# matpalm/cartpoleplusplus

Hardware: AMD Instinct MI355X
Metric: DDPG training steps/sec, 64x64x18 pixel obs, batch=256 (higher is better)
Workload: dtype f32-acc/f16x2,bf16x6

## Files before the change

cartpoleplusplus_amd/csrc/conv_dw16_rs.h:

```cpp
#pragma once
#include <type_traits>
#include "conv_dw16.h"

template <int CIN_>
struct Dw16RsGeom {
  static constexpr int KS = 5, P = 2, PB = 2, CIN = CIN_, NO = KYO_NO, WC = 32, NPC = 2;
  static constexpr int CP0 = (CIN + 1 + 3) & ~3;
  static constexpr int CP = ((CP0 / 2) % 8 == 0) ? CP0 + 4 : CP0;
  static constexpr bool ODD = (CIN & 1) != 0;
  static constexpr int MT = (KS * CP + 15) / 16, NT = (KS * NO + 15) / 16;
  static constexpr int WPX = WC + 2 * P;
  static constexpr int ROWB = 2 * (((CP * WPX + 16 * MT - KS * CP) + 7) & ~7);
  static constexpr int NXS = 2;
  static constexpr int DOST = 80, DPC = NO * DOST;
  static constexpr int DSLOT = NPC * DPC;
  static constexpr int NDS = KS + 1;
  static constexpr int WVB = NXS * ROWB + NDS * DSLOT;
  static constexpr int SUMB = MT * NT * 64 * 16;
  static constexpr int BASEB = 4 * WVB > 2 * SUMB ? 4 * WVB : 2 * SUMB;
  static constexpr int TXB = NT * KS * 16 * 4;
  static constexpr int LDS_BYTES = (BASEB + 4 * TXB + 2 * CIN * 4 + 15) & ~15;
  static constexpr int NW = KS * KS * CIN * NO;
  static_assert(ROWB % 16 == 0 && WVB % 16 == 0 && BASEB % 16 == 0, "16-byte aligned slots");
  static_assert(MT * NT * 4 <= 112, "the accumulators of a unit: at most 112 registers (18 channels); 30 channels would need 160");
};

template <int CIN_>
__device__ __forceinline__ void conv_dw16_rs_body(const ConvArgsN& batch, const int nbands, const int band, const int bx, const int by) {
  typedef Dw16RsGeom<CIN_> G;
  constexpr int KS = G::KS, P = G::P, PB = G::PB, CIN = G::CIN, NO = G::NO, WC = G::WC, CP = G::CP, MT = G::MT, NT = G::NT, NPC = G::NPC;
  constexpr int ROWB = G::ROWB, DOST = G::DOST, DPC = G::DPC, DSLOT = G::DSLOT, NDS = G::NDS;
  constexpr unsigned BIG = 0x08000000u;
  extern __shared__ __attribute__((aligned(16))) unsigned char dw16rs_lds[];
  const int tid = threadIdx.x, lane = tid & 63, li = lane & 15, lj = lane >> 4;
  const int swave = __builtin_amdgcn_readfirstlane(tid >> 6);
  const int net = swave & 1, col = swave >> 1;
  const ConvArgs& a = batch.a[by + net];
  unsigned char* wvb = dw16rs_lds + swave * G::WVB;
  unsigned char* xring = wvb;
  unsigned char* dzring = wvb + G::NXS * ROWB;
  float* wsc = reinterpret_cast<float*>(dw16rs_lds + G::BASEB + 4 * G::TXB);
  const int H = a.H, Hp = H >> 1, W = a.W, Wp = W >> 1, nout = a.nout;
  const int ub = bx / nbands, bd = bx - ub * nbands;
  const int x0 = col * WC;
  const int q_lo = bd * band;
  const int rows = min(band, H - q_lo);
  const int y0 = q_lo - PB;
  if (tid < CIN) { wsc[tid] = a.scale[tid]; wsc[CIN + tid] = a.shift[tid]; }

  for (int i = lane; i < G::WVB / 16; i += 64) reinterpret_cast<k16_u32x4*>(wvb)[i] = (k16_u32x4){0u, 0u, 0u, 0u};
  for (int i = lane; i < G::NXS * G::WPX; i += 64) {
    const int s = i / G::WPX, wx = i - s * G::WPX, x = x0 - P + wx;
    if (x >= 0 && x < W) *reinterpret_cast<unsigned short*>(xring + s * ROWB + 2 * (CP * wx + CIN)) = (unsigned short)0x3C00u;
  }

  constexpr bool ODDC = G::ODD;
  constexpr int NXV = ODDC ? (G::WPX * CIN / 2 + 63) / 64 : (G::WPX * (CIN / 2) + 63) / 64;
  const __amdgpu_buffer_rsrc_t in_rsrc = __builtin_amdgcn_make_buffer_rsrc(
      const_cast<__half*>((const __half*)a.in + (long)(a.img_slot ? a.img_slot[ub] : ub) * a.in_bstride), 0, H * W * CIN * 2, 0x00020000);
  unsigned xvo[NXV]; uint32_t xdst[NXV]; uint32_t xdst_hi[ODDC ? NXV : 1];
#pragma unroll
  for (int i = 0; i < NXV; ++i) {
    const int idx = lane + 64 * i;
    if (!ODDC) {
      const int wx = idx / (CIN / 2), cp = idx - (CIN / 2) * wx;
      const int x = x0 - P + wx;
      const bool on = idx < G::WPX * (CIN / 2);
      xvo[i] = (on && x >= 0 && x < W) ? (unsigned)((x * CIN + 2 * cp) * 2) : BIG;
      xdst[i] = keep_in_vgpr(lds_addr(xring + (on ? 2 * (CP * wx + 2 * cp) : ROWB - 8)));
    } else {
      const int h0 = 2 * idx, h1 = 2 * idx + 1;
      const int wx0 = h0 / CIN, wx1 = h1 / CIN;
      const int x = x0 - P + wx0;
      const bool on = idx < G::WPX * CIN / 2;
      xvo[i] = (on && x >= 0 && x < W) ? (unsigned)(((x0 - P) * CIN + h0) * 2) : BIG;
      xdst[i] = keep_in_vgpr(lds_addr(xring + (on ? 2 * (CP * wx0 + (h0 - CIN * wx0)) : ROWB - 8)));
      xdst_hi[i] = keep_in_vgpr(lds_addr(xring + (on ? 2 * (CP * wx1 + (h1 - CIN * wx1)) : ROWB - 6)));
    }
  }
  unsigned xraw[2][NXV];
  auto x_load = [&](const int buf, const int q) __attribute__((always_inline)) {
    const unsigned ro = q < H ? (unsigned)(q * (W * CIN * 2)) : BIG;
#pragma unroll
    for (int i = 0; i < NXV; ++i) xraw[buf][i] = __builtin_amdgcn_raw_buffer_load_b32(in_rsrc, (int)(xvo[i] + ro), 0, 0);
  };
  auto x_store = [&](const int buf, const int slot) __attribute__((always_inline)) {
#pragma unroll
    for (int i = 0; i < NXV; ++i) {
      if (!ODDC) lds_store(xdst[i], slot * ROWB, xraw[buf][i]);
      else { lds_store_u16(xdst[i], slot * ROWB, xraw[buf][i] & 0xFFFFu); lds_store_u16(xdst_hi[i], slot * ROWB, xraw[buf][i] >> 16); }
    }
  };

  const int zg = lane / NO, zo = lane - zg * NO;
  const bool zon = lane < 4 * NO;
  const __amdgpu_buffer_rsrc_t dp_rsrc = __builtin_amdgcn_make_buffer_rsrc(const_cast<float*>(a.dy.dpool + (long)ub * a.dy.dpool_bstride), 0,
                                                                           Hp * Wp * NO * 4, 0x00020000);
  const __amdgpu_buffer_rsrc_t am_rsrc = __builtin_amdgcn_make_buffer_rsrc(const_cast<uint8_t*>(a.dy.amax + (long)ub * Hp * Wp * NO), 0,
                                                                           Hp * Wp * NO, 0x00020000);
  const unsigned zoff = zon ? (unsigned)((x0 / 2 + 8 * (zg & 1) + (zg >> 1)) * NO + zo) : BIG;
  const uint32_t zdst = keep_in_vgpr(lds_addr(dzring + (zon ? zo * DOST + zg * 16 : DOST - 16)));

  float sc, inv;
  {
    const int pylo = max(0, (q_lo - P) >> 1), pyhi = min(Hp - 1, (q_lo + rows - 1 + P) >> 1);
    float vmax = 0.f;
    if (a.dy.imax) {
      const f32x4 im = *reinterpret_cast<const f32x4*>(a.dy.imax + (long)ub * DX_IMAX_SLOTS), im2 = *reinterpret_cast<const f32x4*>(a.dy.imax + (long)ub * DX_IMAX_SLOTS + 4);
      vmax = fmaxf(fmaxf(fmaxf(im[0], im[1]), fmaxf(im[2], im[3])), fmaxf(fmaxf(im2[0], im2[1]), fmaxf(im2[2], im2[3])));
    }
    constexpr int PSR = 9;
    for (int py = a.dy.imax ? pyhi + 1 : pylo; py <= pyhi; py += PSR) {
      float t[PSR][4];
#pragma unroll
      for (int u = 0; u < PSR; ++u) {
        const unsigned ro = py + u <= pyhi ? (unsigned)((py + u) * (Wp * NO)) : BIG;
#pragma unroll
        for (int j = 0; j < 4; ++j) t[u][j] = __uint_as_float(__builtin_amdgcn_raw_buffer_load_b32(dp_rsrc, (int)((zoff + ro + (unsigned)(2 * j * NO)) * 4u), 0, 0));
      }
#pragma unroll
      for (int u = 0; u < PSR; ++u)
#pragma unroll
        for (int j = 0; j < 4; ++j) vmax = fmaxf(vmax, fabsf(t[u][j]));
    }
    for (int o = 32; o > 0; o >>= 1) vmax = fmaxf(vmax, __shfl_xor(vmax, o));
    int S = 0;
    if (vmax > 0.f && vmax < 3.0e38f) S = 14 - ilogbf(vmax);
    S = S > 100 ? 100 : (S < -100 ? -100 : S);
    sc = ldexpf(1.f, S); inv = ldexpf(1.f, -S);
  }

  float zrg[2][4]; unsigned zrc[2][4];
#pragma unroll
  for (int b = 0; b < 2; ++b)
#pragma unroll
    for (int j = 0; j < 4; ++j) { zrg[b][j] = 0.f; zrc[b][j] = 0u; }
  unsigned zp01[NPC] = {0u, 0u}, zp23[NPC] = {0u, 0u};
  unsigned zm01[4] = {0u, 0u, 0u, 0u}, zm23[4] = {0u, 0u, 0u, 0u};
  auto z_load = [&](const int buf, const int py) __attribute__((always_inline)) {
    const unsigned ro = (py >= 0 && py < Hp) ? (unsigned)(py * (Wp * NO)) : BIG;
#pragma unroll
    for (int j = 0; j < 4; ++j) {
      const unsigned e = zoff + ro + (unsigned)(2 * j * NO);
      zrg[buf][j] = __uint_as_float(__builtin_amdgcn_raw_buffer_load_b32(dp_rsrc, (int)(e * 4u), 0, 0));
      zrc[buf][j] = (unsigned)__builtin_amdgcn_raw_buffer_load_b8(am_rsrc, (int)e, 0, 0);
    }
  };
  auto z_convert_half = [&](const int buf, const int hf) __attribute__((always_inline)) {
    unsigned short pc[2][NPC];
#pragma unroll
    for (int j = 0; j < 2; ++j) {
      const float g = (zrc[buf][2 * hf + j] & POOL_ACTIVE) ? zrg[buf][2 * hf + j] : 0.f;
      const float v = g * sc;
      const _Float16 h = (_Float16)v;
      const _Float16 m = (_Float16)(v - (float)h);
      pc[j][0] = __builtin_bit_cast(unsigned short, h); pc[j][1] = __builtin_bit_cast(unsigned short, m);
    }
#pragma unroll
    for (int p = 0; p < NPC; ++p) {
      const unsigned v = (unsigned)pc[0][p] | ((unsigned)pc[1][p] << 16);
      if (hf == 0) zp01[p] = v; else zp23[p] = v;
    }
#pragma unroll
    for (int pos = 0; pos < 4; ++pos) {
      const unsigned v = ((zrc[buf][2 * hf] & 3u) == (unsigned)pos ? 0xFFFFu : 0u) | ((zrc[buf][2 * hf + 1] & 3u) == (unsigned)pos ? 0xFFFF0000u : 0u);
      if (hf == 0) zm01[pos] = v; else zm23[pos] = v;
    }
  };
  auto z_convert = [&](const int buf) __attribute__((always_inline)) { z_convert_half(buf, 0); z_convert_half(buf, 1); };
  auto z_store = [&](const int slot, const int ry) __attribute__((always_inline)) {
#pragma unroll
    for (int p = 0; p < NPC; ++p)
      lds_store(zdst, slot * DSLOT + p * DPC, (k16_u32x4){zp01[p] & zm01[2 * ry], zp23[p] & zm23[2 * ry], zp01[p] & zm01[2 * ry + 1], zp23[p] & zm23[2 * ry + 1]});
  };

  const int tj = (lane >> 2) & 3, tq = lane & 3;
  const uint32_t aadr = keep_in_vgpr(lds_addr(xring + 2 * (CP * (16 * (lj & 1) + 4 * tj + 2 * (lj >> 1)) + 4 * tq)));
  uint32_t bbase[NT]; int bky[NT];
#pragma unroll
  for (int nt = 0; nt < NT; ++nt) {
    const int n = 16 * nt + li;
    const bool nvalid = n < KS * NO;
    bky[nt] = nvalid ? n / NO : 0;
    bbase[nt] = lds_addr(dzring + (nvalid ? n % NO : 0) * DOST + lj * 16);
  }
  f32x4 acc[MT][NT];
#pragma unroll
  for (int mt = 0; mt < MT; ++mt)
#pragma unroll
    for (int nt = 0; nt < NT; ++nt) acc[mt][nt] = (f32x4){0.f, 0.f, 0.f, 0.f};

  {
    const int py0 = y0 >> 1;
    z_load(0, py0); z_load(1, py0 + 1);
    x_load(0, q_lo); x_load(1, q_lo + 1);
#pragma unroll
    for (int d = 0; d <= PB + P; ++d) {
      if ((d & 1) == 0) { z_convert((d / 2) % 2); z_load((d / 2) % 2, py0 + d / 2 + 2); }
      z_store(d % NDS, d & 1);
    }
    x_store(0, 0);
    x_load(0, q_lo + 2);
    __builtin_amdgcn_sched_barrier(0);

    k16_u32x4 bq[NT][NPC];
    auto a_load = [&](k16_u32x4& dst, const int xs, const int mt) __attribute__((always_inline)) {
      const int off = xs * ROWB + mt * 32;
      const dw16_v4s r0 = __builtin_amdgcn_ds_read_tr16_b64_v4i16(
          reinterpret_cast<__attribute__((address_space(3))) dw16_v4s*>((uintptr_t)(aadr + (uint32_t)off)));
      const dw16_v4s r1 = __builtin_amdgcn_ds_read_tr16_b64_v4i16(
          reinterpret_cast<__attribute__((address_space(3))) dw16_v4s*>((uintptr_t)(aadr + (uint32_t)(off + 2 * CP))));
      const dw16_u32x2 u0 = __builtin_bit_cast(dw16_u32x2, r0), u1 = __builtin_bit_cast(dw16_u32x2, r1);
      dst = (k16_u32x4){u0.x, u0.y, u1.x, u1.y};
    };
    auto step = [&](auto sqtag, const int t) __attribute__((always_inline)) {
      constexpr int SQ = decltype(sqtag)::value;
      constexpr int XS = SQ & 1;
      constexpr int ZPOS = SQ + PB + P + 1;
      constexpr bool ZODD = (ZPOS & 1) != 0;
      constexpr int ZBUF = (ZPOS / 2) % 2;
#pragma unroll
      for (int nt = 0; nt < NT; ++nt) {
        int sl = (SQ + PB + P) % NDS - bky[nt]; sl = sl < 0 ? sl + NDS : sl;
        const uint32_t ad = bbase[nt] + (uint32_t)(sl * DSLOT);
#pragma unroll
        for (int p = 0; p < NPC; ++p) bq[nt][p] = lds_load<k16_u32x4>(ad, p * DPC);
      }
      k16_u32x4 av;
      a_load(av, XS, 0);
#pragma unroll
      for (int mt = 0; mt < MT; ++mt) {
        k16_u32x4 an = av;
        if (mt + 1 < MT) a_load(an, XS, mt + 1);
#pragma unroll
        for (int pc = NPC - 1; pc >= 0; --pc)
#pragma unroll
          for (int nt = 0; nt < NT; ++nt)
            acc[mt][nt] = __builtin_amdgcn_mfma_f32_16x16x32_f16(__builtin_bit_cast(f16x8, av), __builtin_bit_cast(f16x8, bq[nt][pc]), acc[mt][nt], 0, 0, 0);
        constexpr int TL = MT - 1;
        if (mt == (0 < TL ? 0 : TL)) { if (!ZODD) z_convert_half(ZBUF, 0); }
        if (mt == (1 < TL ? 1 : TL)) { if (!ZODD) z_convert_half(ZBUF, 1); }
        if (mt == (2 < TL ? 2 : TL)) z_store(ZPOS % NDS, ZODD ? 1 : 0);
        if (mt == (3 < TL ? 3 : TL)) { if (ZODD) z_load(ZBUF, py0 + (t + PB + P + 1) / 2 + 2); }
        if (mt == (4 < TL ? 4 : TL)) x_store((SQ + 1) & 1, XS ^ 1);
        if (mt == (5 < TL ? 5 : TL)) x_load((SQ + 1) & 1, q_lo + t + 3);
        av = an;
      }
      __builtin_amdgcn_sched_barrier(0);
    };
    for (int t0 = 0; t0 < rows; t0 += 12) {
      if (t0 + 0 < rows) step(std::integral_constant<int, 0>{}, t0 + 0);
      if (t0 + 1 < rows) step(std::integral_constant<int, 1>{}, t0 + 1);
      if (t0 + 2 < rows) step(std::integral_constant<int, 2>{}, t0 + 2);
      if (t0 + 3 < rows) step(std::integral_constant<int, 3>{}, t0 + 3);
      if (t0 + 4 < rows) step(std::integral_constant<int, 4>{}, t0 + 4);
      if (t0 + 5 < rows) step(std::integral_constant<int, 5>{}, t0 + 5);
      if (t0 + 6 < rows) step(std::integral_constant<int, 6>{}, t0 + 6);
      if (t0 + 7 < rows) step(std::integral_constant<int, 7>{}, t0 + 7);
      if (t0 + 8 < rows) step(std::integral_constant<int, 8>{}, t0 + 8);
      if (t0 + 9 < rows) step(std::integral_constant<int, 9>{}, t0 + 9);
      if (t0 + 10 < rows) step(std::integral_constant<int, 10>{}, t0 + 10);
      if (t0 + 11 < rows) step(std::integral_constant<int, 11>{}, t0 + 11);
    }
  }

  __syncthreads();
  float* sum = reinterpret_cast<float*>(dw16rs_lds + net * G::SUMB);
  if (col == 0) {
#pragma unroll
    for (int mt = 0; mt < MT; ++mt)
#pragma unroll
      for (int nt = 0; nt < NT; ++nt)
        *reinterpret_cast<f32x4*>(sum + ((mt * NT + nt) * 64 + lane) * 4) = (f32x4){acc[mt][nt][0] * inv, acc[mt][nt][1] * inv, acc[mt][nt][2] * inv, acc[mt][nt][3] * inv};
  }
  __syncthreads();
  if (col == 0) return;
#pragma unroll
  for (int mt = 0; mt < MT; ++mt)
#pragma unroll
    for (int nt = 0; nt < NT; ++nt) {
      const f32x4 o = *reinterpret_cast<const f32x4*>(sum + ((mt * NT + nt) * 64 + lane) * 4);
#pragma unroll
      for (int r = 0; r < 4; ++r) acc[mt][nt][r] = o[r] + acc[mt][nt][r] * inv;
    }
  float* tx = reinterpret_cast<float*>(dw16rs_lds + G::BASEB + swave * G::TXB);
#pragma unroll
  for (int nt = 0; nt < NT; ++nt)
#pragma unroll
    for (int kx = 0; kx < KS; ++kx) {
      const int m = CP * kx + CIN;
      if (lj == ((m & 15) >> 2)) tx[(nt * KS + kx) * 16 + li] = acc[m >> 4][nt][m & 3];
    }
  __builtin_amdgcn_fence(__ATOMIC_RELEASE, "wavefront");
  __builtin_amdgcn_wave_barrier();
  __builtin_amdgcn_fence(__ATOMIC_ACQUIRE, "wavefront");
  float* part = a.partial + (long)bx * a.pstride;
#pragma unroll
  for (int nt = 0; nt < NT; ++nt) {
    const int n = 16 * nt + li;
    const bool nvalid = n < KS * NO;
    const int nky = nvalid ? n / NO : 0, no = nvalid ? n % NO : 0;
    if (nvalid && no < nout) {
#pragma unroll
      for (int mt = 0; mt < MT; ++mt)
#pragma unroll
        for (int r = 0; r < 4; ++r) {
          const int m = 16 * mt + 4 * lj + r;
          const int kx = m / CP, c = m - kx * CP;
          if (kx < KS && c < CIN) {
            const float t = tx[(nt * KS + kx) * 16 + li];
            part[(nky * (KS * CIN) + kx * CIN + c) * nout + no] = wsc[c] * acc[mt][nt][r] + wsc[CIN + c] * t;
          } else if (kx == P && c == CIN && nky == P) part[G::NW / NO * nout + no] = acc[mt][nt][r];
        }
    }
  }
}

int conv_dw16_rs_dispatch(cpp_ctx* ctx, int cin, int ks, int in_mode, bool dense, const ConvArgsN& a, int* grid, bool* handled);
```

Baseline: 3185.

## Prefetch next-row B/A fragments across steps and simplify dz packing

```diff
diff --git a/cartpoleplusplus_amd/csrc/conv_dw16_rs.h b/cartpoleplusplus_amd/csrc/conv_dw16_rs.h
--- a/cartpoleplusplus_amd/csrc/conv_dw16_rs.h
+++ b/cartpoleplusplus_amd/csrc/conv_dw16_rs.h
@@ -135,8 +135,11 @@
   for (int b = 0; b < 2; ++b)
 #pragma unroll
     for (int j = 0; j < 4; ++j) { zrg[b][j] = 0.f; zrc[b][j] = 0u; }
-  unsigned zp01[NPC] = {0u, 0u}, zp23[NPC] = {0u, 0u};
-  unsigned zm01[4] = {0u, 0u, 0u, 0u}, zm23[4] = {0u, 0u, 0u, 0u};
+  unsigned long long zw[4][NPC];
+#pragma unroll
+  for (int j = 0; j < 4; ++j)
+#pragma unroll
+    for (int p = 0; p < NPC; ++p) zw[j][p] = 0ull;
   auto z_load = [&](const int buf, const int py) __attribute__((always_inline)) {
     const unsigned ro = (py >= 0 && py < Hp) ? (unsigned)(py * (Wp * NO)) : BIG;
 #pragma unroll
@@ -147,43 +150,41 @@
     }
   };
   auto z_convert_half = [&](const int buf, const int hf) __attribute__((always_inline)) {
-    unsigned short pc[2][NPC];
-#pragma unroll
-    for (int j = 0; j < 2; ++j) {
-      const float g = (zrc[buf][2 * hf + j] & POOL_ACTIVE) ? zrg[buf][2 * hf + j] : 0.f;
+#pragma unroll
+    for (int j = 2 * hf; j < 2 * hf + 2; ++j) {
+      const float g = (zrc[buf][j] & POOL_ACTIVE) ? zrg[buf][j] : 0.f;
       const float v = g * sc;
       const _Float16 h = (_Float16)v;
       const _Float16 m = (_Float16)(v - (float)h);
-      pc[j][0] = __builtin_bit_cast(unsigned short, h); pc[j][1] = __builtin_bit_cast(unsigned short, m);
-    }
-#pragma unroll
-    for (int p = 0; p < NPC; ++p) {
-      const unsigned v = (unsigned)pc[0][p] | ((unsigned)pc[1][p] << 16);
-      if (hf == 0) zp01[p] = v; else zp23[p] = v;
-    }
-#pragma unroll
-    for (int pos = 0; pos < 4; ++pos) {
-      const unsigned v = ((zrc[buf][2 * hf] & 3u) == (unsigned)pos ? 0xFFFFu : 0u) | ((zrc[buf][2 * hf + 1] & 3u) == (unsigned)pos ? 0xFFFF0000u : 0u);
-      if (hf == 0) zm01[pos] = v; else zm23[pos] = v;
+      const unsigned sh = (zrc[buf][j] << 4) & 63u;
+      zw[j][0] = (unsigned long long)__builtin_bit_cast(unsigned short, h) << sh;
+      zw[j][1] = (unsigned long long)__builtin_bit_cast(unsigned short, m) << sh;
     }
   };
   auto z_convert = [&](const int buf) __attribute__((always_inline)) { z_convert_half(buf, 0); z_convert_half(buf, 1); };
   auto z_store = [&](const int slot, const int ry) __attribute__((always_inline)) {
 #pragma unroll
-    for (int p = 0; p < NPC; ++p)
-      lds_store(zdst, slot * DSLOT + p * DPC, (k16_u32x4){zp01[p] & zm01[2 * ry], zp23[p] & zm23[2 * ry], zp01[p] & zm01[2 * ry + 1], zp23[p] & zm23[2 * ry + 1]});
+    for (int p = 0; p < NPC; ++p) {
+      unsigned d[4];
+#pragma unroll
+      for (int k = 0; k < 4; ++k) {
+        const int j = 2 * (k & 1), rx = k >> 1;
+        d[k] = __builtin_amdgcn_perm((unsigned)(zw[j + 1][p] >> (32 * ry)), (unsigned)(zw[j][p] >> (32 * ry)), rx ? 0x07060302u : 0x05040100u);
+      }
+      lds_store(zdst, slot * DSLOT + p * DPC, (k16_u32x4){d[0], d[1], d[2], d[3]});
+    }
   };
 
   const int tj = (lane >> 2) & 3, tq = lane & 3;
   const uint32_t aadr = keep_in_vgpr(lds_addr(xring + 2 * (CP * (16 * (lj & 1) + 4 * tj + 2 * (lj >> 1)) + 4 * tq)));
-  uint32_t bbase[NT]; int bky[NT];
+  uint32_t bring[NT];
 #pragma unroll
   for (int nt = 0; nt < NT; ++nt) {
     const int n = 16 * nt + li;
     const bool nvalid = n < KS * NO;
-    bky[nt] = nvalid ? n / NO : 0;
-    bbase[nt] = lds_addr(dzring + (nvalid ? n % NO : 0) * DOST + lj * 16);
-  }
+    bring[nt] = keep_in_vgpr(lds_addr(dzring + (NDS - (nvalid ? n / NO : 0)) * DSLOT + (nvalid ? n % NO : 0) * DOST + lj * 16));
+  }
+  const uint32_t bend = lds_addr(dzring + NDS * DSLOT);
   f32x4 acc[MT][NT];
 #pragma unroll
   for (int mt = 0; mt < MT; ++mt)
@@ -201,9 +202,14 @@
     }
     x_store(0, 0);
     x_load(0, q_lo + 2);
-    __builtin_amdgcn_sched_barrier(0);
-
-    k16_u32x4 bq[NT][NPC];
+
+    k16_u32x4 bq[NT][NPC], av;
+    auto b_load = [&](const int sq, const int nt) __attribute__((always_inline)) {
+      const uint32_t c = bring[nt] + (uint32_t)(((sq + PB + P) % NDS) * DSLOT);
+      const uint32_t ad = c >= bend ? c - (uint32_t)(NDS * DSLOT) : c;
+#pragma unroll
+      for (int p = 0; p < NPC; ++p) bq[nt][p] = lds_load<k16_u32x4>(ad, p * DPC);
+    };
     auto a_load = [&](k16_u32x4& dst, const int xs, const int mt) __attribute__((always_inline)) {
       const int off = xs * ROWB + mt * 32;
       const dw16_v4s r0 = __builtin_amdgcn_ds_read_tr16_b64_v4i16(
@@ -213,37 +219,57 @@
       const dw16_u32x2 u0 = __builtin_bit_cast(dw16_u32x2, r0), u1 = __builtin_bit_cast(dw16_u32x2, r1);
       dst = (k16_u32x4){u0.x, u0.y, u1.x, u1.y};
     };
+#pragma unroll
+    for (int nt = 0; nt < NT; ++nt) b_load(0, nt);
+    a_load(av, 0, 0);
+    __builtin_amdgcn_sched_barrier(0);
+
+    auto mfma = [&](const int mt, const int nt, const int pc) __attribute__((always_inline)) {
+      acc[mt][nt] = __builtin_amdgcn_mfma_f32_16x16x32_f16(__builtin_bit_cast(f16x8, av), __builtin_bit_cast(f16x8, bq[nt][pc]), acc[mt][nt], 0, 0, 0);
+    };
     auto step = [&](auto sqtag, const int t) __attribute__((always_inline)) {
       constexpr int SQ = decltype(sqtag)::value;
       constexpr int XS = SQ & 1;
       constexpr int ZPOS = SQ + PB + P + 1;
       constexpr bool ZODD = (ZPOS & 1) != 0;
       constexpr int ZBUF = (ZPOS / 2) % 2;
-#pragma unroll
-      for (int nt = 0; nt < NT; ++nt) {
-        int sl = (SQ + PB + P) % NDS - bky[nt]; sl = sl < 0 ? sl + NDS : sl;
-        const uint32_t ad = bbase[nt] + (uint32_t)(sl * DSLOT);
-#pragma unroll
-        for (int p = 0; p < NPC; ++p) bq[nt][p] = lds_load<k16_u32x4>(ad, p * DPC);
-      }
-      k16_u32x4 av;
-      a_load(av, XS, 0);
-#pragma unroll
-      for (int mt = 0; mt < MT; ++mt) {
-        k16_u32x4 an = av;
-        if (mt + 1 < MT) a_load(an, XS, mt + 1);
-#pragma unroll
-        for (int pc = NPC - 1; pc >= 0; --pc)
-#pragma unroll
-          for (int nt = 0; nt < NT; ++nt)
-            acc[mt][nt] = __builtin_amdgcn_mfma_f32_16x16x32_f16(__builtin_bit_cast(f16x8, av), __builtin_bit_cast(f16x8, bq[nt][pc]), acc[mt][nt], 0, 0, 0);
-        constexpr int TL = MT - 1;
+      constexpr int TL = MT - 1;
+      auto stage = [&](const int mt) __attribute__((always_inline)) {
         if (mt == (0 < TL ? 0 : TL)) { if (!ZODD) z_convert_half(ZBUF, 0); }
         if (mt == (1 < TL ? 1 : TL)) { if (!ZODD) z_convert_half(ZBUF, 1); }
         if (mt == (2 < TL ? 2 : TL)) z_store(ZPOS % NDS, ZODD ? 1 : 0);
         if (mt == (3 < TL ? 3 : TL)) { if (ZODD) z_load(ZBUF, py0 + (t + PB + P + 1) / 2 + 2); }
         if (mt == (4 < TL ? 4 : TL)) x_store((SQ + 1) & 1, XS ^ 1);
         if (mt == (5 < TL ? 5 : TL)) x_load((SQ + 1) & 1, q_lo + t + 3);
+      };
+#pragma unroll
+      for (int mt = 0; mt < TL; ++mt) {
+        k16_u32x4 an;
+        a_load(an, XS, mt + 1);
+        if (mt == 0) {
+#pragma unroll
+          for (int nt = 0; nt < NT; ++nt)
+#pragma unroll
+            for (int pc = NPC - 1; pc >= 0; --pc) mfma(mt, nt, pc);
+        } else {
+#pragma unroll
+          for (int pc = NPC - 1; pc >= 0; --pc)
+#pragma unroll
+            for (int nt = 0; nt < NT; ++nt) mfma(mt, nt, pc);
+        }
+        stage(mt);
+        av = an;
+      }
+      stage(TL);
+      {
+        k16_u32x4 an;
+        a_load(an, XS ^ 1, 0);
+#pragma unroll
+        for (int nt = 0; nt < NT; ++nt) {
+#pragma unroll
+          for (int pc = NPC - 1; pc >= 0; --pc) mfma(TL, nt, pc);
+          b_load((SQ + 1) % 12, nt);
+        }
         av = an;
       }
       __builtin_amdgcn_sched_barrier(0);
```

Result: no change. 3198, median of 6 (+0.4%).
